# KKKSQJ/DeepLearning

Measured on AMD Instinct MI355X. Metric: images/sec, higher is better.
Workload: dtype bf16; 1 GPU; model=resnet50, global_batch=256, image_size=224, parallelism=dp1

## Files before the change

csrc/batchnorm.hip:

```cpp
#include "common.h"
#include "vec.h"

namespace dla {

__device__ __forceinline__ float bn_pre(float x, float sc, float sh) {
  return fmaf(x, sc, sh);
}

template <typename dev_t>
__global__ void bn_stats_kernel(const dev_t* __restrict__ x, float* __restrict__ sums,
                                int N, int C, int64_t HW) {
  __shared__ float smem[16];
  const int c = blockIdx.x;
  const int64_t total = (int64_t)N * HW;
  float sum = 0.f, sumsq = 0.f;
  for (int64_t m = (int64_t)blockIdx.y * blockDim.x + threadIdx.x; m < total;
       m += (int64_t)gridDim.y * blockDim.x) {
    const int64_t n = m / HW, hw = m % HW;
    const float f = to_f32(x[(n * C + c) * HW + hw]);
    sum += f;
    sumsq += f * f;
  }
  sum = block_reduce_sum(sum, smem);
  sumsq = block_reduce_sum(sumsq, smem);
// ... 153 lines not shown
    const float m_dyxh = sums[C + c] * inv_count;
    dx[i] = from_f32<dev_t>(weight[c] * rs * (g - m_dy - xh * m_dyxh));
  }
}



inline int64_t nhwc_used_threads(int lanes_per_row, int64_t rows,
                                 int64_t target_lanes) {
  int64_t k = target_lanes / lanes_per_row;
  if (k > rows) k = rows;
  if (k < 1) k = 1;
  return (int64_t)lanes_per_row * k;
}

template <typename dev_t, int V>
__global__ void bn_stats_nhwc_kernel(const dev_t* __restrict__ x,
                                     float* __restrict__ sums, int C,
                                     int64_t rows, int64_t used) {
  extern __shared__ float ls[];
  for (int i = threadIdx.x; i < 2 * C; i += blockDim.x) ls[i] = 0.f;
  __syncthreads();
  const int64_t t = (int64_t)blockIdx.x * blockDim.x + threadIdx.x;
  const int lanes_per_row = C / V;
  if (t < used) {
    const int c0 = (int)(t % lanes_per_row) * V;
    const int64_t rstride = used / lanes_per_row;
    float s[V], q[V];
#pragma unroll
    for (int j = 0; j < V; ++j) { s[j] = 0.f; q[j] = 0.f; }
    for (int64_t r = t / lanes_per_row; r < rows; r += rstride) {
      Vec<dev_t, V> xv = vload<dev_t, V>(x + r * C + c0);
#pragma unroll
      for (int j = 0; j < V; ++j) {
        const float f = to_f32(xv.v[j]);
        s[j] += f;
        q[j] += f * f;
      }
    }
#pragma unroll
    for (int j = 0; j < V; ++j) {
      atomicAdd(&ls[c0 + j], s[j]);
      atomicAdd(&ls[C + c0 + j], q[j]);
    }
  }
  __syncthreads();
  for (int i = threadIdx.x; i < 2 * C; i += blockDim.x)
    atomicAdd(&sums[i], ls[i]);
}

template <typename dev_t, int V, bool RELU>
__global__ void bn_apply_nhwc_kernel(const dev_t* __restrict__ x,
                                     const float* __restrict__ scale,
                                     const float* __restrict__ shift,
                                     dev_t* __restrict__ y, int C, int64_t rows,
                                     int64_t used) {
  const int64_t t = (int64_t)blockIdx.x * blockDim.x + threadIdx.x;
  if (t >= used) return;
  const int lanes_per_row = C / V;
  const int c0 = (int)(t % lanes_per_row) * V;
  const int64_t rstride = used / lanes_per_row;
  float sc[V], sh[V];
#pragma unroll
  for (int j = 0; j < V; ++j) { sc[j] = scale[c0 + j]; sh[j] = shift[c0 + j]; }
  for (int64_t r = t / lanes_per_row; r < rows; r += rstride) {
    Vec<dev_t, V> xv = vload<dev_t, V>(x + r * C + c0);
    Vec<dev_t, V> yv;
#pragma unroll
    for (int j = 0; j < V; ++j) {
      const float f = bn_pre(to_f32(xv.v[j]), sc[j], sh[j]);
      yv.v[j] = from_f32<dev_t>(RELU ? fmaxf(f, 0.f) : f);
    }
    vstore<dev_t, V>(y + r * C + c0, yv);
  }
}

template <typename dev_t, int V, bool RELU, bool MASK_Y = false>
__global__ void bn_bwd_stats_nhwc_kernel(const dev_t* __restrict__ dy,
                                         const dev_t* __restrict__ x,
                                         const dev_t* __restrict__ y,
                                         const float* __restrict__ scale,
                                         const float* __restrict__ shift,
                                         const float* __restrict__ mean,
                                         const float* __restrict__ rstd,
                                         float* __restrict__ sums, int C,
                                         int64_t rows, int64_t used) {
  extern __shared__ float ls[];
  for (int i = threadIdx.x; i < 2 * C; i += blockDim.x) ls[i] = 0.f;
  __syncthreads();
  const int64_t t = (int64_t)blockIdx.x * blockDim.x + threadIdx.x;
  const int lanes_per_row = C / V;
  if (t < used) {
    const int c0 = (int)(t % lanes_per_row) * V;
    const int64_t rstride = used / lanes_per_row;
    float mu[V], rs[V], sc[V], sh[V], s_dy[V], s_dyxh[V];
#pragma unroll
    for (int j = 0; j < V; ++j) {
      mu[j] = mean[c0 + j];
      rs[j] = rstd[c0 + j];
      sc[j] = (RELU && !MASK_Y) ? scale[c0 + j] : 0.f;
      sh[j] = (RELU && !MASK_Y) ? shift[c0 + j] : 0.f;
      s_dy[j] = 0.f;
      s_dyxh[j] = 0.f;
    }
    for (int64_t r = t / lanes_per_row; r < rows; r += rstride) {
      const int64_t base = r * C + c0;
      Vec<dev_t, V> dyv = vload<dev_t, V>(dy + base);
      Vec<dev_t, V> xv = vload<dev_t, V>(x + base);
      Vec<dev_t, V> yv;
      if (RELU && MASK_Y) yv = vload<dev_t, V>(y + base);
#pragma unroll
      for (int j = 0; j < V; ++j) {
        float g = to_f32(dyv.v[j]);
        const float xf = to_f32(xv.v[j]);
        if (RELU && MASK_Y && to_f32(yv.v[j]) <= 0.f) g = 0.f;
        if (RELU && !MASK_Y && !(bn_pre(xf, sc[j], sh[j]) > 0.f)) g = 0.f;
        const float xh = (xf - mu[j]) * rs[j];
        s_dy[j] += g;
        s_dyxh[j] += g * xh;
      }
    }
#pragma unroll
    for (int j = 0; j < V; ++j) {
      atomicAdd(&ls[c0 + j], s_dy[j]);
      atomicAdd(&ls[C + c0 + j], s_dyxh[j]);
    }
  }
  __syncthreads();
  for (int i = threadIdx.x; i < 2 * C; i += blockDim.x)
    atomicAdd(&sums[i], ls[i]);
}

template <typename dev_t, int V, bool RELU, bool MASK_Y = false>
__global__ void bn_bwd_dx_nhwc_kernel(const dev_t* __restrict__ dy,
                                      const dev_t* __restrict__ x,
                                      const dev_t* __restrict__ y,
                                      const float* __restrict__ scale,
                                      const float* __restrict__ shift,
                                      const float* __restrict__ mean,
                                      const float* __restrict__ rstd,
                                      const float* __restrict__ weight,
                                      const float* __restrict__ sums,
                                      dev_t* __restrict__ dx, int C,
                                      int64_t rows, int64_t used,
                                      float inv_count) {
// ... 61 lines not shown
    const int64_t base = r * C + c0;
    Vec<dev_t, V> xv = vload<dev_t, V>(x + base);
    Vec<dev_t, V> iv = vload<dev_t, V>(idn + base);
    Vec<dev_t, V> ov;
#pragma unroll
    for (int j = 0; j < V; ++j) {
      float f = to_f32(xv.v[j]) * sc[j] + sh[j];
      f += DUAL ? to_f32(iv.v[j]) * scd[j] : to_f32(iv.v[j]);
      ov.v[j] = from_f32<dev_t>(fmaxf(f, 0.f));
    }
    vstore<dev_t, V>(out + base, ov);
  }
}

template <typename dev_t, int V, bool DUAL>
__global__ void bn_join_bwd_stats_nhwc_kernel(
    const dev_t* __restrict__ dy, const dev_t* __restrict__ out,
    const dev_t* __restrict__ x, const float* __restrict__ mean,
    const float* __restrict__ rstd, const dev_t* __restrict__ xd,
    const float* __restrict__ mean_d, const float* __restrict__ rstd_d,
    dev_t* __restrict__ g_out, float* __restrict__ sums, int C, int64_t rows,
    int64_t used) {
  constexpr int NS = DUAL ? 3 : 2;
  extern __shared__ float ls[];
  for (int i = threadIdx.x; i < NS * C; i += blockDim.x) ls[i] = 0.f;
  __syncthreads();
  const int64_t t = (int64_t)blockIdx.x * blockDim.x + threadIdx.x;
  const int lanes_per_row = C / V;
  if (t < used) {
    const int c0 = (int)(t % lanes_per_row) * V;
    const int64_t rstride = used / lanes_per_row;
    float mu[V], rs[V], mud[V], rsd[V], s_g[V], s_gxh[V], s_gxhd[V];
#pragma unroll
    for (int j = 0; j < V; ++j) {
      mu[j] = mean[c0 + j];
      rs[j] = rstd[c0 + j];
      mud[j] = DUAL ? mean_d[c0 + j] : 0.f;
      rsd[j] = DUAL ? rstd_d[c0 + j] : 0.f;
      s_g[j] = 0.f;
      s_gxh[j] = 0.f;
      s_gxhd[j] = 0.f;
    }
    for (int64_t r = t / lanes_per_row; r < rows; r += rstride) {
      const int64_t base = r * C + c0;
      Vec<dev_t, V> dyv = vload<dev_t, V>(dy + base);
      Vec<dev_t, V> ov = vload<dev_t, V>(out + base);
      Vec<dev_t, V> xv = vload<dev_t, V>(x + base);
      Vec<dev_t, V> xdv;
      if (DUAL) xdv = vload<dev_t, V>(xd + base);
      Vec<dev_t, V> gv;
#pragma unroll
      for (int j = 0; j < V; ++j) {
        const bool on = to_f32(ov.v[j]) > 0.f;
        gv.v[j] = on ? dyv.v[j] : from_f32<dev_t>(0.f);
        const float g = on ? to_f32(dyv.v[j]) : 0.f;
        s_g[j] += g;
        s_gxh[j] += g * ((to_f32(xv.v[j]) - mu[j]) * rs[j]);
        if (DUAL) s_gxhd[j] += g * ((to_f32(xdv.v[j]) - mud[j]) * rsd[j]);
      }
      vstore<dev_t, V>(g_out + base, gv);
    }
#pragma unroll
    for (int j = 0; j < V; ++j) {
      atomicAdd(&ls[c0 + j], s_g[j]);
      atomicAdd(&ls[C + c0 + j], s_gxh[j]);
      if (DUAL) atomicAdd(&ls[2 * C + c0 + j], s_gxhd[j]);
    }
  }
  __syncthreads();
  for (int i = threadIdx.x; i < NS * C; i += blockDim.x)
    atomicAdd(&sums[i], ls[i]);
}

template <typename dev_t, int V>
__global__ void bn_join_bwd_dx_dual_nhwc_kernel(
    const dev_t* __restrict__ g, const dev_t* __restrict__ x,
    const dev_t* __restrict__ xd, const float* __restrict__ mean,
    const float* __restrict__ rstd, const float* __restrict__ weight,
    const float* __restrict__ mean_d, const float* __restrict__ rstd_d,
    const float* __restrict__ weight_d, const float* __restrict__ sums,
    dev_t* __restrict__ dx, dev_t* __restrict__ dxd, int C, int64_t rows,
    int64_t used, float inv_count) {
  const int64_t t = (int64_t)blockIdx.x * blockDim.x + threadIdx.x;
  if (t >= used) return;
  const int lanes_per_row = C / V;
  const int c0 = (int)(t % lanes_per_row) * V;
// ... 74 lines not shown
    hipLaunchKernelGGL(bn_finalize_kernel, dim3((C + 255) / 256), dim3(256), 0,
                       stream(), sums.data_ptr<float>(), w32.data_ptr<float>(),
                       b32.data_ptr<float>(), f.mean.data_ptr<float>(),
                       f.rstd.data_ptr<float>(), rm, rv,
                       f.scale.data_ptr<float>(), f.shift.data_ptr<float>(), C,
                       (float)rows, (float)eps, (float)momentum);
  }
  return f;
}

inline torch::Tensor bn_param_grad(const torch::Tensor& sums, int64_t offset,
                                   int C, const torch::Tensor& weight) {
  return sums.narrow(0, offset, C).to(weight.scalar_type());
}

inline bool is_nhwc_rows(const torch::Tensor& t) {
  return t.dim() == 4 && t.is_contiguous(at::MemoryFormat::ChannelsLast);
}

}

std::vector<torch::Tensor> batchnorm_fwd(torch::Tensor x, torch::Tensor weight,
                                         torch::Tensor bias,
                                         c10::optional<torch::Tensor> running_mean,
                                         c10::optional<torch::Tensor> running_var,
                                         double momentum, double eps, bool relu) {
  DLA_CHECK_CUDA(x);
  TORCH_CHECK(x.dim() == 4, "batchnorm_fwd expects a 4D tensor");
  const bool nhwc = dla::is_nhwc(x);
  TORCH_CHECK(nhwc || x.is_contiguous(), "batchnorm_fwd: x must be contiguous "
              "(NCHW or channels_last)");
  const int N = (int)x.size(0), C = (int)x.size(1);
  const int64_t HW = x.size(2) * x.size(3);
  auto opts_f = x.options().dtype(torch::kFloat);
  auto sums = torch::zeros({2 * C}, opts_f);
  auto mean = torch::empty({C}, opts_f);
  auto rstd = torch::empty({C}, opts_f);
  auto scale = torch::empty({C}, opts_f);
  auto shift = torch::empty({C}, opts_f);
  auto y = torch::empty_like(x);
  auto w32 = weight.to(torch::kFloat);
  auto b32 = bias.to(torch::kFloat);

  const int64_t rows = (int64_t)N * HW;
  const int ysplit = (int)std::min<int64_t>((rows + 65535) / 65536 + 1,
                                            std::max(1, 2048 / C));
  DLA_DISPATCH_FLOAT_TYPES(x.scalar_type(), "batchnorm_fwd", [&] {
    if (nhwc) {
      constexpr int VM = 16 / (int)sizeof(dev_t);
      auto stats = [&](auto vtag) {
        constexpr int V = decltype(vtag)::value;
        const int lanes = C / V;
        const int64_t used = dla::nhwc_used_threads(lanes, rows, 262144);
        const int lds = 2 * C * sizeof(float);
        hipLaunchKernelGGL((dla::bn_stats_nhwc_kernel<dev_t, V>),
                           dim3((int)((used + 255) / 256)), dim3(256), lds,
                           dla::stream(), (const dev_t*)x.data_ptr(),
                           sums.data_ptr<float>(), C, rows, used);
      };
      if (C % VM == 0) stats(std::integral_constant<int, VM>{});
      else if (C % 2 == 0) stats(std::integral_constant<int, 2>{});
      else stats(std::integral_constant<int, 1>{});
    } else {
      hipLaunchKernelGGL((dla::bn_stats_kernel<dev_t>), dim3(C, ysplit), dim3(256), 0,
                         dla::stream(), (const dev_t*)x.data_ptr(),
                         sums.data_ptr<float>(), N, C, HW);
    }
    hipLaunchKernelGGL(dla::bn_finalize_kernel, dim3((C + 255) / 256), dim3(256), 0,
                       dla::stream(), sums.data_ptr<float>(), w32.data_ptr<float>(),
                       b32.data_ptr<float>(), mean.data_ptr<float>(),
                       rstd.data_ptr<float>(),
                       running_mean.has_value() ? running_mean->data_ptr<float>() : nullptr,
                       running_var.has_value() ? running_var->data_ptr<float>() : nullptr,
                       scale.data_ptr<float>(), shift.data_ptr<float>(), C,
                       (float)rows, (float)eps, (float)momentum);
    const int64_t n_total = x.numel();
    constexpr int VMAX = 16 / (int)sizeof(dev_t);
    auto launch = [&](auto vtag, auto rtag) {
      constexpr int V = decltype(vtag)::value;
      constexpr bool R = decltype(rtag)::value;
      if (nhwc) {
        const int lanes = C / V;
        const int64_t used = dla::nhwc_used_threads(lanes, rows, 524288);
        hipLaunchKernelGGL((dla::bn_apply_nhwc_kernel<dev_t, V, R>),
                           dim3((int)((used + 255) / 256)), dim3(256), 0,
                           dla::stream(), (const dev_t*)x.data_ptr(),
                           scale.data_ptr<float>(), shift.data_ptr<float>(),
                           (dev_t*)y.data_ptr(), C, rows, used);
        return;
      }
// ... 127 lines not shown

std::vector<torch::Tensor> batchnorm_bwd_ex(
    torch::Tensor dy, torch::Tensor x, c10::optional<torch::Tensor> y,
    torch::Tensor weight, torch::Tensor mean, torch::Tensor rstd,
    c10::optional<torch::Tensor> scale, c10::optional<torch::Tensor> shift,
    bool relu) {
  DLA_CHECK_CUDA(dy); DLA_CHECK_CUDA(x);
  const bool nhwc = dla::is_nhwc(x);
  TORCH_CHECK(nhwc || x.is_contiguous(), "batchnorm_bwd: x must be contiguous");
  if (nhwc && !dla::is_nhwc(dy)) dy = dy.contiguous(at::MemoryFormat::ChannelsLast);
  if (!nhwc) dy = dy.contiguous();
  const int N = (int)x.size(0), C = (int)x.size(1);
  const int64_t HW = x.size(2) * x.size(3);
  const int64_t rows = (int64_t)N * HW;
  auto opts_f = x.options().dtype(torch::kFloat);
  auto sums = torch::zeros({2 * C}, opts_f);
  auto dx = torch::empty_like(x);
  auto w32 = weight.to(torch::kFloat);
  const int ysplit = (int)std::min<int64_t>((rows + 65535) / 65536 + 1,
                                            std::max(1, 2048 / C));
  const bool mask_y = relu && y.has_value();
  if (relu && !mask_y) {
    TORCH_CHECK(bn_relu_mask_from_x(x) && scale.has_value() && shift.has_value(),
                "batchnorm_bwd: the relu mask needs y, or channels_last x "
                "with the forward's scale and shift");
    for (const auto* t : {&*scale, &*shift})
      TORCH_CHECK(t->is_cuda() && t->scalar_type() == torch::kFloat &&
                      t->is_contiguous() && t->numel() == C,
                  "batchnorm_bwd: scale/shift must be contiguous fp32 [C]");
  }
  if (mask_y)
// ... 4 lines not shown
  const float* shp = (relu && !mask_y) ? shift->data_ptr<float>() : nullptr;
  DLA_DISPATCH_FLOAT_TYPES(x.scalar_type(), "batchnorm_bwd", [&] {
    const dev_t* yp = mask_y ? (const dev_t*)y->data_ptr() : nullptr;
    auto with_mode = [&](auto f) {
      if (!relu) f(std::false_type{}, std::false_type{});
      else if (mask_y) f(std::true_type{}, std::true_type{});
      else f(std::true_type{}, std::false_type{});
    };
    with_mode([&](auto rtag, auto mtag) {
      constexpr bool R = decltype(rtag)::value;
      constexpr bool MY = decltype(mtag)::value;
      if (nhwc) {
        constexpr int VM = 16 / (int)sizeof(dev_t);
        auto stats = [&](auto vtag) {
          constexpr int V = decltype(vtag)::value;
          const int lanes = C / V;
          const int64_t used = dla::nhwc_used_threads(lanes, rows, 262144);
          const int lds = 2 * C * sizeof(float);
          hipLaunchKernelGGL((dla::bn_bwd_stats_nhwc_kernel<dev_t, V, R, MY>),
                             dim3((int)((used + 255) / 256)), dim3(256), lds,
                             dla::stream(), (const dev_t*)dy.data_ptr(),
                             (const dev_t*)x.data_ptr(), yp, scp, shp,
                             mean.data_ptr<float>(), rstd.data_ptr<float>(),
                             sums.data_ptr<float>(), C, rows, used);
        };
        if (C % VM == 0) stats(std::integral_constant<int, VM>{});
        else if (C % 2 == 0) stats(std::integral_constant<int, 2>{});
        else stats(std::integral_constant<int, 1>{});
      } else if constexpr (!R || MY) {
        hipLaunchKernelGGL((dla::bn_bwd_stats_kernel<dev_t, R>), dim3(C, ysplit),
                           dim3(256), 0, dla::stream(), (const dev_t*)dy.data_ptr(),
                           (const dev_t*)x.data_ptr(), yp, mean.data_ptr<float>(),
                           rstd.data_ptr<float>(), sums.data_ptr<float>(), N, C, HW);
      }
    });

    const int64_t n_total = x.numel();
    const float inv_count = 1.f / (float)rows;
    constexpr int VMAX = 16 / (int)sizeof(dev_t);
// ... 121 lines not shown

std::vector<torch::Tensor> bn_add_relu_bwd(torch::Tensor dy, torch::Tensor out,
                                           torch::Tensor x, torch::Tensor weight,
                                           torch::Tensor mean,
                                           torch::Tensor rstd) {
  DLA_CHECK_CUDA(x);
  TORCH_CHECK(dla::is_nhwc_rows(x), "bn_add_relu_bwd: x must be channels_last");
  dla::join_check(x, out, "out");
  if (!dla::is_nhwc_rows(dy)) dy = dy.contiguous(at::MemoryFormat::ChannelsLast);
  dla::join_check(x, dy, "dy");
  dla::join_vec(x);
  const int C = (int)x.size(1);
  const int64_t rows = x.numel() / C;
  TORCH_CHECK(mean.numel() == C && rstd.numel() == C && weight.numel() == C,
              "bn_add_relu_bwd: per-channel tensors must have C elements");
  auto sums = torch::zeros({2 * C}, x.options().dtype(torch::kFloat));
  auto g = torch::empty_like(x);
  auto dx = torch::empty_like(x);
  auto w32 = weight.to(torch::kFloat).contiguous();
  DLA_DISPATCH_FLOAT_TYPES(x.scalar_type(), "bn_add_relu_bwd", [&] {
    constexpr int V = 16 / (int)sizeof(dev_t);
    const int lanes = C / V;
    const int64_t used_s = dla::nhwc_used_threads(lanes, rows, 262144);
    hipLaunchKernelGGL((dla::bn_join_bwd_stats_nhwc_kernel<dev_t, V, false>),
                       dim3((int)((used_s + 255) / 256)), dim3(256),
                       2 * C * sizeof(float), dla::stream(),
                       (const dev_t*)dy.data_ptr(), (const dev_t*)out.data_ptr(),
                       (const dev_t*)x.data_ptr(), mean.data_ptr<float>(),
                       rstd.data_ptr<float>(), nullptr, nullptr, nullptr,
                       (dev_t*)g.data_ptr(), sums.data_ptr<float>(), C, rows,
                       used_s);
    const int64_t used = dla::nhwc_used_threads(lanes, rows, 524288);
    hipLaunchKernelGGL((dla::bn_bwd_dx_nhwc_kernel<dev_t, V, false>),
                       dim3((int)((used + 255) / 256)), dim3(256), 0,
                       dla::stream(), (const dev_t*)g.data_ptr(),
                       (const dev_t*)x.data_ptr(), nullptr, nullptr, nullptr,
                       mean.data_ptr<float>(), rstd.data_ptr<float>(),
                       w32.data_ptr<float>(), sums.data_ptr<float>(),
                       (dev_t*)dx.data_ptr(), C, rows, used,
                       1.f / (float)rows);
  });
  HIP_CHECK_ERR();
  return {g, dx, dla::bn_param_grad(sums, C, C, weight),
          dla::bn_param_grad(sums, 0, C, weight)};
}

// ... 2 lines not shown
    torch::Tensor mean, torch::Tensor rstd, torch::Tensor xd,
    torch::Tensor weight_d, torch::Tensor mean_d, torch::Tensor rstd_d) {
  DLA_CHECK_CUDA(x);
  TORCH_CHECK(dla::is_nhwc_rows(x), "bn_add_relu_dual_bwd: x must be channels_last");
  dla::join_check(x, out, "out");
  dla::join_check(x, xd, "xd");
  if (!dla::is_nhwc_rows(dy)) dy = dy.contiguous(at::MemoryFormat::ChannelsLast);
  dla::join_check(x, dy, "dy");
  dla::join_vec(x);
  const int C = (int)x.size(1);
  const int64_t rows = x.numel() / C;
  TORCH_CHECK(mean.numel() == C && rstd.numel() == C && weight.numel() == C &&
                  mean_d.numel() == C && rstd_d.numel() == C &&
                  weight_d.numel() == C,
              "bn_add_relu_dual_bwd: per-channel tensors must have C elements");
  auto sums = torch::zeros({3 * C}, x.options().dtype(torch::kFloat));
  auto g = torch::empty_like(x);
  auto dx = torch::empty_like(x);
  auto dxd = torch::empty_like(x);
  auto w32 = weight.to(torch::kFloat).contiguous();
  auto wd32 = weight_d.to(torch::kFloat).contiguous();
  DLA_DISPATCH_FLOAT_TYPES(x.scalar_type(), "bn_add_relu_dual_bwd", [&] {
    constexpr int V = 16 / (int)sizeof(dev_t);
    const int lanes = C / V;
    const int64_t used_s = dla::nhwc_used_threads(lanes, rows, 262144);
    hipLaunchKernelGGL((dla::bn_join_bwd_stats_nhwc_kernel<dev_t, V, true>),
                       dim3((int)((used_s + 255) / 256)), dim3(256),
                       3 * C * sizeof(float), dla::stream(),
                       (const dev_t*)dy.data_ptr(), (const dev_t*)out.data_ptr(),
                       (const dev_t*)x.data_ptr(), mean.data_ptr<float>(),
                       rstd.data_ptr<float>(), (const dev_t*)xd.data_ptr(),
                       mean_d.data_ptr<float>(), rstd_d.data_ptr<float>(),
                       (dev_t*)g.data_ptr(), sums.data_ptr<float>(), C, rows,
                       used_s);
    const int64_t used = dla::nhwc_used_threads(lanes, rows, 524288);
    hipLaunchKernelGGL((dla::bn_join_bwd_dx_dual_nhwc_kernel<dev_t, V>),
                       dim3((int)((used + 255) / 256)), dim3(256), 0,
                       dla::stream(), (const dev_t*)g.data_ptr(),
                       (const dev_t*)x.data_ptr(), (const dev_t*)xd.data_ptr(),
                       mean.data_ptr<float>(), rstd.data_ptr<float>(),
                       w32.data_ptr<float>(), mean_d.data_ptr<float>(),
                       rstd_d.data_ptr<float>(), wd32.data_ptr<float>(),
                       sums.data_ptr<float>(), (dev_t*)dx.data_ptr(),
                       (dev_t*)dxd.data_ptr(), C, rows, used,
                       1.f / (float)rows);
  });
  HIP_CHECK_ERR();
  auto dbias = dla::bn_param_grad(sums, 0, C, weight);
  return {dx, dxd, dla::bn_param_grad(sums, C, C, weight), dbias,
// ... 81 lines not shown
    for (int ow = w >> 1; ow <= ow_hi; ++ow) {
      const int want = kh * 3 + (w - 2 * ow + 1);
      const int64_t o = (((int64_t)n * OH + oh) * OW + ow) * C + c0;
      Vec<uint8_t, V> sv = vload<uint8_t, V>(slots + o);
      Vec<dev_t, V> dv = vload<dev_t, V>(dpool + o);
#pragma unroll
      for (int j = 0; j < V; ++j)
        if ((int)sv.v[j] == want) g[j] += to_f32(dv.v[j]);
    }
  }
#pragma unroll
  for (int j = 0; j < V; ++j)
    if (!(bn_pre(to_f32(xv.v[j]), sc[j], sh[j]) > 0.f)) g[j] = 0.f;
}

template <typename dev_t, int V>
__global__ void bn_relu_maxpool_bwd_stats_nhwc_kernel(
    const dev_t* __restrict__ dpool, const uint8_t* __restrict__ slots,
    const dev_t* __restrict__ x, const float* __restrict__ scale,
    const float* __restrict__ shift, const float* __restrict__ mean,
    const float* __restrict__ rstd, float* __restrict__ sums, int C, int H,
    int W, int OH, int OW, int64_t rows, int64_t used) {
  extern __shared__ float ls[];
  for (int i = threadIdx.x; i < 2 * C; i += blockDim.x) ls[i] = 0.f;
  __syncthreads();
  const int64_t t = (int64_t)blockIdx.x * blockDim.x + threadIdx.x;
  const int lanes_per_row = C / V;
  if (t < used) {
    const int c0 = (int)(t % lanes_per_row) * V;
    const int64_t rstride = used / lanes_per_row;
    float mu[V], rs[V], sc[V], sh[V], s_g[V], s_gxh[V], g[V];
#pragma unroll
    for (int j = 0; j < V; ++j) {
      mu[j] = mean[c0 + j];
      rs[j] = rstd[c0 + j];
      sc[j] = scale[c0 + j];
      sh[j] = shift[c0 + j];
      s_g[j] = 0.f;
      s_gxh[j] = 0.f;
    }
    for (int64_t r = t / lanes_per_row; r < rows; r += rstride) {
      const uint32_t r32 = (uint32_t)r;
      const uint32_t q = r32 / (uint32_t)W;
      const int w = (int)(r32 - q * (uint32_t)W);
      const int n = (int)(q / (uint32_t)H);
      const int h = (int)(q - (uint32_t)n * (uint32_t)H);
      Vec<dev_t, V> xv = vload<dev_t, V>(x + r * C + c0);
      stem_pool_grad<dev_t, V>(dpool, slots, xv, sc, sh, n, h, w, c0, C, OH,
                               OW, g);
#pragma unroll
      for (int j = 0; j < V; ++j) {
        const float xh = (to_f32(xv.v[j]) - mu[j]) * rs[j];
        s_g[j] += g[j];
        s_gxh[j] += g[j] * xh;
      }
    }
#pragma unroll
    for (int j = 0; j < V; ++j) {
      atomicAdd(&ls[c0 + j], s_g[j]);
      atomicAdd(&ls[C + c0 + j], s_gxh[j]);
    }
  }
  __syncthreads();
  for (int i = threadIdx.x; i < 2 * C; i += blockDim.x)
    atomicAdd(&sums[i], ls[i]);
}

template <typename dev_t, int V>
__global__ void bn_relu_maxpool_bwd_dx_nhwc_kernel(
    const dev_t* __restrict__ dpool, const uint8_t* __restrict__ slots,
    const dev_t* __restrict__ x, const float* __restrict__ scale,
    const float* __restrict__ shift, const float* __restrict__ mean,
    const float* __restrict__ rstd, const float* __restrict__ weight,
    const float* __restrict__ sums, dev_t* __restrict__ dx, int C, int H,
    int W, int OH, int OW, int64_t rows, int64_t used, float inv_count) {
  const int64_t t = (int64_t)blockIdx.x * blockDim.x + threadIdx.x;
  if (t >= used) return;
  const int lanes_per_row = C / V;
  const int c0 = (int)(t % lanes_per_row) * V;
  const int64_t rstride = used / lanes_per_row;
// ... 35 lines not shown
  TORCH_CHECK(x.numel() > 0 && x.numel() / x.size(1) < (int64_t(1) << 31),
              fn, ": N*H*W must be in [1, 2^31)");
}

}

std::vector<torch::Tensor> bn_relu_maxpool_fwd(
    torch::Tensor x, torch::Tensor weight, torch::Tensor bias,
    c10::optional<torch::Tensor> running_mean,
    c10::optional<torch::Tensor> running_var, double momentum, double eps) {
  dla::stem_check(x, "bn_relu_maxpool_fwd");
  const int N = (int)x.size(0), C = (int)x.size(1);
  const int H = (int)x.size(2), W = (int)x.size(3);
  const int OH = (H - 1) / 2 + 1, OW = (W - 1) / 2 + 1;
  const int64_t rows = (int64_t)N * H * W;
  auto sums = torch::zeros({2 * C}, x.options().dtype(torch::kFloat));
  auto out_opts = x.options().memory_format(at::MemoryFormat::ChannelsLast);
  auto pooled = torch::empty({N, C, OH, OW}, out_opts);
  auto slots = torch::empty({N, C, OH, OW}, out_opts.dtype(torch::kByte));
  const int runs = (OH + dla::kPoolRun - 1) / dla::kPoolRun;
  TORCH_CHECK((int64_t)N * runs < (int64_t(1) << 31),
              "bn_relu_maxpool_fwd: too many blocks");
  dla::BnFinalized fin;
  DLA_DISPATCH_FLOAT_TYPES(x.scalar_type(), "bn_relu_maxpool_fwd", [&] {
    constexpr int V = 16 / (int)sizeof(dev_t);
    const int64_t used = dla::nhwc_used_threads(C / V, rows, 262144);
    hipLaunchKernelGGL((dla::bn_stats_nhwc_kernel<dev_t, V>),
                       dim3((int)((used + 255) / 256)), dim3(256),
                       2 * C * sizeof(float), dla::stream(),
                       (const dev_t*)x.data_ptr(), sums.data_ptr<float>(), C,
                       rows, used);
    fin = dla::bn_finalize_launch(sums, weight, bias, running_mean,
                                  running_var, C, rows, momentum, eps);
    hipLaunchKernelGGL((dla::bn_relu_maxpool_fwd_nhwc_kernel<dev_t, V>),
                       dim3(N * runs), dim3(256), 0, dla::stream(),
                       (const dev_t*)x.data_ptr(), fin.scale.data_ptr<float>(),
                       fin.shift.data_ptr<float>(), (dev_t*)pooled.data_ptr(),
                       slots.data_ptr<uint8_t>(), C, H, W, OH, OW, runs);
  });
  HIP_CHECK_ERR();
  return {pooled, slots, fin.mean, fin.rstd, fin.scale, fin.shift};
}

std::vector<torch::Tensor> bn_relu_maxpool_bwd(
    torch::Tensor dpool, torch::Tensor x, torch::Tensor slots,
    torch::Tensor weight, torch::Tensor mean, torch::Tensor rstd,
// ... 9 lines not shown
  const std::vector<int64_t> pshape{N, C, OH, OW};
  TORCH_CHECK(dpool.scalar_type() == x.scalar_type() &&
                  dpool.sizes() == at::IntArrayRef(pshape),
              "bn_relu_maxpool_bwd: dpool must be [N, C, OH, OW] of x's dtype");
  TORCH_CHECK(slots.is_cuda() && slots.scalar_type() == torch::kByte &&
                  slots.sizes() == at::IntArrayRef(pshape) &&
                  dla::is_nhwc_rows(slots),
              "bn_relu_maxpool_bwd: slots must be channels_last uint8 "
              "[N, C, OH, OW]");
  for (const auto* t : {&mean, &rstd, &scale, &shift})
    TORCH_CHECK(t->is_cuda() && t->scalar_type() == torch::kFloat &&
                    t->is_contiguous() && t->numel() == C,
                "bn_relu_maxpool_bwd: per-channel tensors must be contiguous "
                "fp32 [C]");
  TORCH_CHECK(weight.numel() == C, "bn_relu_maxpool_bwd: weight must be [C]");
  auto sums = torch::zeros({2 * C}, x.options().dtype(torch::kFloat));
  auto dx = torch::empty_like(x);
  auto w32 = weight.to(torch::kFloat).contiguous();
  DLA_DISPATCH_FLOAT_TYPES(x.scalar_type(), "bn_relu_maxpool_bwd", [&] {
    constexpr int V = 16 / (int)sizeof(dev_t);
    const int lanes = C / V;
    const int64_t used_s = dla::nhwc_used_threads(lanes, rows, 262144);
    hipLaunchKernelGGL((dla::bn_relu_maxpool_bwd_stats_nhwc_kernel<dev_t, V>),
                       dim3((int)((used_s + 255) / 256)), dim3(256),
                       2 * C * sizeof(float), dla::stream(),
                       (const dev_t*)dpool.data_ptr(),
                       slots.data_ptr<uint8_t>(), (const dev_t*)x.data_ptr(),
                       scale.data_ptr<float>(), shift.data_ptr<float>(),
                       mean.data_ptr<float>(), rstd.data_ptr<float>(),
                       sums.data_ptr<float>(), C, H, W, OH, OW, rows, used_s);
    const int64_t used = dla::nhwc_used_threads(lanes, rows, 524288);
    hipLaunchKernelGGL((dla::bn_relu_maxpool_bwd_dx_nhwc_kernel<dev_t, V>),
                       dim3((int)((used + 255) / 256)), dim3(256), 0,
                       dla::stream(), (const dev_t*)dpool.data_ptr(),
                       slots.data_ptr<uint8_t>(), (const dev_t*)x.data_ptr(),
                       scale.data_ptr<float>(), shift.data_ptr<float>(),
                       mean.data_ptr<float>(), rstd.data_ptr<float>(),
                       w32.data_ptr<float>(), sums.data_ptr<float>(),
                       (dev_t*)dx.data_ptr(), C, H, W, OH, OW, rows, used,
                       1.f / (float)rows);
  });
  HIP_CHECK_ERR();
  return {dx, dla::bn_param_grad(sums, C, C, weight),
          dla::bn_param_grad(sums, 0, C, weight)};
}
// ... 1 lines not shown
```

Before: 9196 images/s.

## Replace atomic BN channel reductions with two-stage slab reduction

```diff
diff --git a/csrc/batchnorm.hip b/csrc/batchnorm.hip
--- a/csrc/batchnorm.hip
+++ b/csrc/batchnorm.hip
@@ -191,39 +191,138 @@
   return (int64_t)lanes_per_row * k;
 }
 
+constexpr int kRedThreads = 256;
+constexpr int kRedLanes = 32;
+constexpr int kRedBlocks = 2048;
+constexpr int kRedMaxParts = 512;
+constexpr int kRedMinRows = 8;
+constexpr int red_unroll(int tensors) { return tensors <= 2 ? 4 : 2; }
+
+#define DLA_RED_KERNEL \
+  __launch_bounds__(dla::kRedThreads) __attribute__((amdgpu_waves_per_eu(1, 4)))
+
+struct NhwcRedTile {
+  int bl, rb, chunks, parts;
+};
+
+inline NhwcRedTile nhwc_red_tile(int lanes_per_row, int64_t rows,
+                                 int blocks = kRedBlocks,
+                                 int max_parts = kRedMaxParts) {
+  NhwcRedTile t;
+  t.chunks = (lanes_per_row + kRedLanes - 1) / kRedLanes;
+  t.bl = (lanes_per_row + t.chunks - 1) / t.chunks;
+  t.rb = kRedThreads / t.bl;
+  const int64_t per_part = (int64_t)t.rb * kRedMinRows;
+  const int64_t by_rows = (rows + per_part - 1) / per_part;
+  const int64_t p = std::min<int64_t>(
+      std::min<int64_t>(blocks / t.chunks, max_parts), by_rows);
+  t.parts = (int)std::max<int64_t>(p, 1);
+  return t;
+}
+
+struct NhwcRedPos {
+  int c0;
+  int64_t row;
+  int64_t rstride;
+  bool active;
+};
+
+template <int V>
+__device__ __forceinline__ NhwcRedPos nhwc_red_pos(int C, int bl, int rb) {
+  const int lane = threadIdx.x % bl, rl = threadIdx.x / bl;
+  const int gl = blockIdx.x * bl + lane;
+  NhwcRedPos p;
+  p.c0 = gl * V;
+  p.row = (int64_t)blockIdx.y * rb + rl;
+  p.rstride = (int64_t)gridDim.y * rb;
+  p.active = rl < rb && gl < C / V;
+  return p;
+}
+
+template <int U, typename L, typename A>
+__device__ __forceinline__ void nhwc_red_rows(const NhwcRedPos& p,
+                                              int64_t rows, L&& load, A&& add) {
+  if (!p.active) return;
+  using D = decltype(load(int64_t{}));
+  int64_t r = p.row;
+  for (; r + (U - 1) * p.rstride < rows; r += U * p.rstride) {
+    D d[U];
+#pragma unroll
+    for (int u = 0; u < U; ++u) d[u] = load(r + u * p.rstride);
+#pragma unroll
+    for (int u = 0; u < U; ++u) add(r + u * p.rstride, d[u]);
+  }
+  for (; r < rows; r += p.rstride) add(r, load(r));
+}
+
+template <int V, int NS>
+__device__ __forceinline__ void nhwc_red_tail(const float (&acc)[NS][V],
+                                              float* __restrict__ slab, int C,
+                                              int bl, int rb) {
+  __shared__ __attribute__((aligned(16))) float ls[kRedThreads * V];
+  const int W = bl * V;
+  const int cbase = blockIdx.x * W;
+  float* out = slab + (int64_t)blockIdx.y * NS * C;
+#pragma unroll
+  for (int s = 0; s < NS; ++s) {
+    if (s) __syncthreads();
+    if ((int)threadIdx.x < bl * rb) {
+#pragma unroll
+      for (int j = 0; j < V; ++j) ls[threadIdx.x * V + j] = acc[s][j];
+    }
+    __syncthreads();
+    for (int col = threadIdx.x; col < W; col += kRedThreads) {
+      if (cbase + col < C) {
+        float sum = 0.f;
+        for (int r = 0; r < rb; ++r) sum += ls[r * W + col];
+        out[s * C + cbase + col] = sum;
+      }
+    }
+  }
+}
+
+constexpr int kSlabCols = 32, kSlabRows = 32;
+
+__global__ void __launch_bounds__(kSlabCols * kSlabRows)
+bn_slab_reduce_kernel(const float* __restrict__ slab, int n_parts, int n_cols,
+                      float* __restrict__ sums) {
+  __shared__ float ls[kSlabRows][kSlabCols + 1];
+  const int cl = threadIdx.x % kSlabCols, rl = threadIdx.x / kSlabCols;
+  const int c = blockIdx.x * kSlabCols + cl;
+  float s = 0.f;
+  if (c < n_cols) {
+#pragma unroll 4
+    for (int r = rl; r < n_parts; r += kSlabRows)
+      s += slab[(int64_t)r * n_cols + c];
+  }
+  ls[rl][cl] = s;
+  __syncthreads();
+  for (int h = kSlabRows / 2; h > 0; h >>= 1) {
+    if (rl < h) ls[rl][cl] += ls[rl + h][cl];
+    __syncthreads();
+  }
+  if (rl == 0 && c < n_cols) sums[c] = ls[0][cl];
+}
+
 template <typename dev_t, int V>
-__global__ void bn_stats_nhwc_kernel(const dev_t* __restrict__ x,
-                                     float* __restrict__ sums, int C,
-                                     int64_t rows, int64_t used) {
-  extern __shared__ float ls[];
-  for (int i = threadIdx.x; i < 2 * C; i += blockDim.x) ls[i] = 0.f;
-  __syncthreads();
-  const int64_t t = (int64_t)blockIdx.x * blockDim.x + threadIdx.x;
-  const int lanes_per_row = C / V;
-  if (t < used) {
-    const int c0 = (int)(t % lanes_per_row) * V;
-    const int64_t rstride = used / lanes_per_row;
-    float s[V], q[V];
-#pragma unroll
-    for (int j = 0; j < V; ++j) { s[j] = 0.f; q[j] = 0.f; }
-    for (int64_t r = t / lanes_per_row; r < rows; r += rstride) {
-      Vec<dev_t, V> xv = vload<dev_t, V>(x + r * C + c0);
-#pragma unroll
-      for (int j = 0; j < V; ++j) {
-        const float f = to_f32(xv.v[j]);
-        s[j] += f;
-        q[j] += f * f;
-      }
-    }
-#pragma unroll
-    for (int j = 0; j < V; ++j) {
-      atomicAdd(&ls[c0 + j], s[j]);
-      atomicAdd(&ls[C + c0 + j], q[j]);
-    }
-  }
-  __syncthreads();
-  for (int i = threadIdx.x; i < 2 * C; i += blockDim.x)
-    atomicAdd(&sums[i], ls[i]);
+__global__ void DLA_RED_KERNEL
+bn_stats_nhwc_kernel(const dev_t* __restrict__ x, float* __restrict__ slab,
+                     int C, int64_t rows, int bl, int rb) {
+  const NhwcRedPos p = nhwc_red_pos<V>(C, bl, rb);
+  float acc[2][V];
+#pragma unroll
+  for (int j = 0; j < V; ++j) { acc[0][j] = 0.f; acc[1][j] = 0.f; }
+  nhwc_red_rows<red_unroll(1)>(
+      p, rows, [&](int64_t r) { return vload<dev_t, V>(x + r * C + p.c0); },
+      [&](int64_t, const Vec<dev_t, V>& xv) {
+#pragma unroll
+        for (int j = 0; j < V; ++j) {
+          const float f = to_f32(xv.v[j]);
+          acc[0][j] += f;
+          acc[1][j] += f * f;
+        }
+      });
+  nhwc_red_tail<V, 2>(acc, slab, C, bl, rb);
 }
 
 template <typename dev_t, int V, bool RELU>
@@ -253,59 +352,54 @@
 }
 
 template <typename dev_t, int V, bool RELU, bool MASK_Y = false>
-__global__ void bn_bwd_stats_nhwc_kernel(const dev_t* __restrict__ dy,
-                                         const dev_t* __restrict__ x,
-                                         const dev_t* __restrict__ y,
-                                         const float* __restrict__ scale,
-                                         const float* __restrict__ shift,
-                                         const float* __restrict__ mean,
-                                         const float* __restrict__ rstd,
-                                         float* __restrict__ sums, int C,
-                                         int64_t rows, int64_t used) {
-  extern __shared__ float ls[];
-  for (int i = threadIdx.x; i < 2 * C; i += blockDim.x) ls[i] = 0.f;
-  __syncthreads();
-  const int64_t t = (int64_t)blockIdx.x * blockDim.x + threadIdx.x;
-  const int lanes_per_row = C / V;
-  if (t < used) {
-    const int c0 = (int)(t % lanes_per_row) * V;
-    const int64_t rstride = used / lanes_per_row;
-    float mu[V], rs[V], sc[V], sh[V], s_dy[V], s_dyxh[V];
-#pragma unroll
-    for (int j = 0; j < V; ++j) {
-      mu[j] = mean[c0 + j];
-      rs[j] = rstd[c0 + j];
-      sc[j] = (RELU && !MASK_Y) ? scale[c0 + j] : 0.f;
-      sh[j] = (RELU && !MASK_Y) ? shift[c0 + j] : 0.f;
-      s_dy[j] = 0.f;
-      s_dyxh[j] = 0.f;
-    }
-    for (int64_t r = t / lanes_per_row; r < rows; r += rstride) {
-      const int64_t base = r * C + c0;
-      Vec<dev_t, V> dyv = vload<dev_t, V>(dy + base);
-      Vec<dev_t, V> xv = vload<dev_t, V>(x + base);
-      Vec<dev_t, V> yv;
-      if (RELU && MASK_Y) yv = vload<dev_t, V>(y + base);
-#pragma unroll
-      for (int j = 0; j < V; ++j) {
-        float g = to_f32(dyv.v[j]);
-        const float xf = to_f32(xv.v[j]);
-        if (RELU && MASK_Y && to_f32(yv.v[j]) <= 0.f) g = 0.f;
-        if (RELU && !MASK_Y && !(bn_pre(xf, sc[j], sh[j]) > 0.f)) g = 0.f;
-        const float xh = (xf - mu[j]) * rs[j];
-        s_dy[j] += g;
-        s_dyxh[j] += g * xh;
-      }
-    }
-#pragma unroll
-    for (int j = 0; j < V; ++j) {
-      atomicAdd(&ls[c0 + j], s_dy[j]);
-      atomicAdd(&ls[C + c0 + j], s_dyxh[j]);
-    }
-  }
-  __syncthreads();
-  for (int i = threadIdx.x; i < 2 * C; i += blockDim.x)
-    atomicAdd(&sums[i], ls[i]);
+__global__ void DLA_RED_KERNEL
+bn_bwd_stats_nhwc_kernel(const dev_t* __restrict__ dy,
+                         const dev_t* __restrict__ x,
+                         const dev_t* __restrict__ y,
+                         const float* __restrict__ scale,
+                         const float* __restrict__ shift,
+                         const float* __restrict__ mean,
+                         const float* __restrict__ rstd,
+                         float* __restrict__ slab, int C, int64_t rows, int bl,
+                         int rb) {
+  const NhwcRedPos p = nhwc_red_pos<V>(C, bl, rb);
+  float mu[V], rs[V], sc[V], sh[V];
+  float acc[2][V];
+#pragma unroll
+  for (int j = 0; j < V; ++j) {
+    mu[j] = p.active ? mean[p.c0 + j] : 0.f;
+    rs[j] = p.active ? rstd[p.c0 + j] : 0.f;
+    sc[j] = (p.active && RELU && !MASK_Y) ? scale[p.c0 + j] : 0.f;
+    sh[j] = (p.active && RELU && !MASK_Y) ? shift[p.c0 + j] : 0.f;
+    acc[0][j] = 0.f;
+    acc[1][j] = 0.f;
+  }
+  struct Row {
+    Vec<dev_t, V> dy, x, y;
+  };
+  nhwc_red_rows<red_unroll(MASK_Y ? 3 : 2)>(
+      p, rows,
+      [&](int64_t r) {
+        const int64_t base = r * C + p.c0;
+        Row d;
+        d.dy = vload<dev_t, V>(dy + base);
+        d.x = vload<dev_t, V>(x + base);
+        if (RELU && MASK_Y) d.y = vload<dev_t, V>(y + base);
+        return d;
+      },
+      [&](int64_t, const Row& d) {
+#pragma unroll
+        for (int j = 0; j < V; ++j) {
+          float g = to_f32(d.dy.v[j]);
+          const float xf = to_f32(d.x.v[j]);
+          if (RELU && MASK_Y && to_f32(d.y.v[j]) <= 0.f) g = 0.f;
+          if (RELU && !MASK_Y && !(bn_pre(xf, sc[j], sh[j]) > 0.f)) g = 0.f;
+          const float xh = (xf - mu[j]) * rs[j];
+          acc[0][j] += g;
+          acc[1][j] += g * xh;
+        }
+      });
+  nhwc_red_tail<V, 2>(acc, slab, C, bl, rb);
 }
 
 template <typename dev_t, int V, bool RELU, bool MASK_Y = false>
@@ -397,62 +491,56 @@
 }
 
 template <typename dev_t, int V, bool DUAL>
-__global__ void bn_join_bwd_stats_nhwc_kernel(
+__global__ void DLA_RED_KERNEL
+bn_join_bwd_stats_nhwc_kernel(
     const dev_t* __restrict__ dy, const dev_t* __restrict__ out,
     const dev_t* __restrict__ x, const float* __restrict__ mean,
     const float* __restrict__ rstd, const dev_t* __restrict__ xd,
     const float* __restrict__ mean_d, const float* __restrict__ rstd_d,
-    dev_t* __restrict__ g_out, float* __restrict__ sums, int C, int64_t rows,
-    int64_t used) {
+    dev_t* __restrict__ g_out, float* __restrict__ slab, int C, int64_t rows,
+    int bl, int rb) {
   constexpr int NS = DUAL ? 3 : 2;
-  extern __shared__ float ls[];
-  for (int i = threadIdx.x; i < NS * C; i += blockDim.x) ls[i] = 0.f;
-  __syncthreads();
-  const int64_t t = (int64_t)blockIdx.x * blockDim.x + threadIdx.x;
-  const int lanes_per_row = C / V;
-  if (t < used) {
-    const int c0 = (int)(t % lanes_per_row) * V;
-    const int64_t rstride = used / lanes_per_row;
-    float mu[V], rs[V], mud[V], rsd[V], s_g[V], s_gxh[V], s_gxhd[V];
-#pragma unroll
-    for (int j = 0; j < V; ++j) {
-      mu[j] = mean[c0 + j];
-      rs[j] = rstd[c0 + j];
-      mud[j] = DUAL ? mean_d[c0 + j] : 0.f;
-      rsd[j] = DUAL ? rstd_d[c0 + j] : 0.f;
-      s_g[j] = 0.f;
-      s_gxh[j] = 0.f;
-      s_gxhd[j] = 0.f;
-    }
-    for (int64_t r = t / lanes_per_row; r < rows; r += rstride) {
-      const int64_t base = r * C + c0;
-      Vec<dev_t, V> dyv = vload<dev_t, V>(dy + base);
-      Vec<dev_t, V> ov = vload<dev_t, V>(out + base);
-      Vec<dev_t, V> xv = vload<dev_t, V>(x + base);
-      Vec<dev_t, V> xdv;
-      if (DUAL) xdv = vload<dev_t, V>(xd + base);
-      Vec<dev_t, V> gv;
-#pragma unroll
-      for (int j = 0; j < V; ++j) {
-        const bool on = to_f32(ov.v[j]) > 0.f;
-        gv.v[j] = on ? dyv.v[j] : from_f32<dev_t>(0.f);
-        const float g = on ? to_f32(dyv.v[j]) : 0.f;
-        s_g[j] += g;
-        s_gxh[j] += g * ((to_f32(xv.v[j]) - mu[j]) * rs[j]);
-        if (DUAL) s_gxhd[j] += g * ((to_f32(xdv.v[j]) - mud[j]) * rsd[j]);
-      }
-      vstore<dev_t, V>(g_out + base, gv);
-    }
-#pragma unroll
-    for (int j = 0; j < V; ++j) {
-      atomicAdd(&ls[c0 + j], s_g[j]);
-      atomicAdd(&ls[C + c0 + j], s_gxh[j]);
-      if (DUAL) atomicAdd(&ls[2 * C + c0 + j], s_gxhd[j]);
-    }
-  }
-  __syncthreads();
-  for (int i = threadIdx.x; i < NS * C; i += blockDim.x)
-    atomicAdd(&sums[i], ls[i]);
+  const NhwcRedPos p = nhwc_red_pos<V>(C, bl, rb);
+  float mu[V], rs[V], mud[V], rsd[V];
+  float acc[NS][V];
+#pragma unroll
+  for (int j = 0; j < V; ++j) {
+    mu[j] = p.active ? mean[p.c0 + j] : 0.f;
+    rs[j] = p.active ? rstd[p.c0 + j] : 0.f;
+    mud[j] = (p.active && DUAL) ? mean_d[p.c0 + j] : 0.f;
+    rsd[j] = (p.active && DUAL) ? rstd_d[p.c0 + j] : 0.f;
+#pragma unroll
+    for (int s = 0; s < NS; ++s) acc[s][j] = 0.f;
+  }
+  struct Row {
+    Vec<dev_t, V> dy, out, x, xd;
+  };
+  nhwc_red_rows<red_unroll(DUAL ? 4 : 3)>(
+      p, rows,
+      [&](int64_t r) {
+        const int64_t base = r * C + p.c0;
+        Row d;
+        d.dy = vload<dev_t, V>(dy + base);
+        d.out = vload<dev_t, V>(out + base);
+        d.x = vload<dev_t, V>(x + base);
+        if (DUAL) d.xd = vload<dev_t, V>(xd + base);
+        return d;
+      },
+      [&](int64_t r, const Row& d) {
+        Vec<dev_t, V> gv;
+#pragma unroll
+        for (int j = 0; j < V; ++j) {
+          const bool on = to_f32(d.out.v[j]) > 0.f;
+          gv.v[j] = on ? d.dy.v[j] : from_f32<dev_t>(0.f);
+          const float g = on ? to_f32(d.dy.v[j]) : 0.f;
+          acc[0][j] += g;
+          acc[1][j] += g * ((to_f32(d.x.v[j]) - mu[j]) * rs[j]);
+          if (DUAL)
+            acc[NS - 1][j] += g * ((to_f32(d.xd.v[j]) - mud[j]) * rsd[j]);
+        }
+        vstore<dev_t, V>(g_out + r * C + p.c0, gv);
+      });
+  nhwc_red_tail<V, NS>(acc, slab, C, bl, rb);
 }
 
 template <typename dev_t, int V>
@@ -557,6 +645,17 @@
   return sums.narrow(0, offset, C).to(weight.scalar_type());
 }
 
+inline torch::Tensor bn_slab_reduce_launch(const torch::Tensor& slab) {
+  const int n_parts = (int)slab.size(0), n_cols = (int)slab.size(1);
+  auto sums = torch::empty({n_cols}, slab.options());
+  hipLaunchKernelGGL(bn_slab_reduce_kernel,
+                     dim3((n_cols + kSlabCols - 1) / kSlabCols),
+                     dim3(kSlabCols * kSlabRows), 0, stream(),
+                     slab.data_ptr<float>(), n_parts, n_cols,
+                     sums.data_ptr<float>());
+  return sums;
+}
+
 inline bool is_nhwc_rows(const torch::Tensor& t) {
   return t.dim() == 4 && t.is_contiguous(at::MemoryFormat::ChannelsLast);
 }
@@ -576,7 +675,7 @@
   const int N = (int)x.size(0), C = (int)x.size(1);
   const int64_t HW = x.size(2) * x.size(3);
   auto opts_f = x.options().dtype(torch::kFloat);
-  auto sums = torch::zeros({2 * C}, opts_f);
+  auto sums = nhwc ? torch::Tensor() : torch::zeros({2 * C}, opts_f);
   auto mean = torch::empty({C}, opts_f);
   auto rstd = torch::empty({C}, opts_f);
   auto scale = torch::empty({C}, opts_f);
@@ -593,13 +692,12 @@
       constexpr int VM = 16 / (int)sizeof(dev_t);
       auto stats = [&](auto vtag) {
         constexpr int V = decltype(vtag)::value;
-        const int lanes = C / V;
-        const int64_t used = dla::nhwc_used_threads(lanes, rows, 262144);
-        const int lds = 2 * C * sizeof(float);
+        const auto t = dla::nhwc_red_tile(C / V, rows);
+        sums = torch::empty({t.parts, 2 * C}, opts_f);
         hipLaunchKernelGGL((dla::bn_stats_nhwc_kernel<dev_t, V>),
-                           dim3((int)((used + 255) / 256)), dim3(256), lds,
+                           dim3(t.chunks, t.parts), dim3(dla::kRedThreads), 0,
                            dla::stream(), (const dev_t*)x.data_ptr(),
-                           sums.data_ptr<float>(), C, rows, used);
+                           sums.data_ptr<float>(), C, rows, t.bl, t.rb);
       };
       if (C % VM == 0) stats(std::integral_constant<int, VM>{});
       else if (C % 2 == 0) stats(std::integral_constant<int, 2>{});
@@ -609,14 +707,25 @@
                          dla::stream(), (const dev_t*)x.data_ptr(),
                          sums.data_ptr<float>(), N, C, HW);
     }
-    hipLaunchKernelGGL(dla::bn_finalize_kernel, dim3((C + 255) / 256), dim3(256), 0,
-                       dla::stream(), sums.data_ptr<float>(), w32.data_ptr<float>(),
-                       b32.data_ptr<float>(), mean.data_ptr<float>(),
-                       rstd.data_ptr<float>(),
-                       running_mean.has_value() ? running_mean->data_ptr<float>() : nullptr,
-                       running_var.has_value() ? running_var->data_ptr<float>() : nullptr,
-                       scale.data_ptr<float>(), shift.data_ptr<float>(), C,
-                       (float)rows, (float)eps, (float)momentum);
+    float* rm = running_mean.has_value() ? running_mean->data_ptr<float>() : nullptr;
+    float* rv = running_var.has_value() ? running_var->data_ptr<float>() : nullptr;
+    if (sums.dim() == 2 && sums.size(0) > 1) {
+      hipLaunchKernelGGL(dla::bn_finalize_parts_kernel,
+                         dim3((C + dla::kFinCh - 1) / dla::kFinCh),
+                         dim3(dla::kFinCh * dla::kFinRows), 0, dla::stream(),
+                         sums.data_ptr<float>(), (int)sums.size(0),
+                         w32.data_ptr<float>(), b32.data_ptr<float>(),
+                         mean.data_ptr<float>(), rstd.data_ptr<float>(), rm, rv,
+                         scale.data_ptr<float>(), shift.data_ptr<float>(), C,
+                         (float)rows, (float)eps, (float)momentum);
+    } else {
+      hipLaunchKernelGGL(dla::bn_finalize_kernel, dim3((C + 255) / 256), dim3(256), 0,
+                         dla::stream(), sums.data_ptr<float>(), w32.data_ptr<float>(),
+                         b32.data_ptr<float>(), mean.data_ptr<float>(),
+                         rstd.data_ptr<float>(), rm, rv,
+                         scale.data_ptr<float>(), shift.data_ptr<float>(), C,
+                         (float)rows, (float)eps, (float)momentum);
+    }
     const int64_t n_total = x.numel();
     constexpr int VMAX = 16 / (int)sizeof(dev_t);
     auto launch = [&](auto vtag, auto rtag) {
@@ -774,7 +883,7 @@
   const int64_t HW = x.size(2) * x.size(3);
   const int64_t rows = (int64_t)N * HW;
   auto opts_f = x.options().dtype(torch::kFloat);
-  auto sums = torch::zeros({2 * C}, opts_f);
+  auto sums = nhwc ? torch::Tensor() : torch::zeros({2 * C}, opts_f);
   auto dx = torch::empty_like(x);
   auto w32 = weight.to(torch::kFloat);
   const int ysplit = (int)std::min<int64_t>((rows + 65535) / 65536 + 1,
@@ -809,15 +918,15 @@
         constexpr int VM = 16 / (int)sizeof(dev_t);
         auto stats = [&](auto vtag) {
           constexpr int V = decltype(vtag)::value;
-          const int lanes = C / V;
-          const int64_t used = dla::nhwc_used_threads(lanes, rows, 262144);
-          const int lds = 2 * C * sizeof(float);
+          const auto t = dla::nhwc_red_tile(C / V, rows);
+          auto slab = torch::empty({t.parts, 2 * C}, opts_f);
           hipLaunchKernelGGL((dla::bn_bwd_stats_nhwc_kernel<dev_t, V, R, MY>),
-                             dim3((int)((used + 255) / 256)), dim3(256), lds,
-                             dla::stream(), (const dev_t*)dy.data_ptr(),
+                             dim3(t.chunks, t.parts), dim3(dla::kRedThreads),
+                             0, dla::stream(), (const dev_t*)dy.data_ptr(),
                              (const dev_t*)x.data_ptr(), yp, scp, shp,
                              mean.data_ptr<float>(), rstd.data_ptr<float>(),
-                             sums.data_ptr<float>(), C, rows, used);
+                             slab.data_ptr<float>(), C, rows, t.bl, t.rb);
+          sums = dla::bn_slab_reduce_launch(slab);
         };
         if (C % VM == 0) stats(std::integral_constant<int, VM>{});
         else if (C % 2 == 0) stats(std::integral_constant<int, 2>{});
@@ -969,22 +1078,25 @@
   const int64_t rows = x.numel() / C;
   TORCH_CHECK(mean.numel() == C && rstd.numel() == C && weight.numel() == C,
               "bn_add_relu_bwd: per-channel tensors must have C elements");
-  auto sums = torch::zeros({2 * C}, x.options().dtype(torch::kFloat));
+  torch::Tensor sums;
   auto g = torch::empty_like(x);
   auto dx = torch::empty_like(x);
   auto w32 = weight.to(torch::kFloat).contiguous();
   DLA_DISPATCH_FLOAT_TYPES(x.scalar_type(), "bn_add_relu_bwd", [&] {
     constexpr int V = 16 / (int)sizeof(dev_t);
     const int lanes = C / V;
-    const int64_t used_s = dla::nhwc_used_threads(lanes, rows, 262144);
+    const auto t = dla::nhwc_red_tile(lanes, rows);
+    auto slab = torch::empty({t.parts, 2 * C},
+                             x.options().dtype(torch::kFloat));
     hipLaunchKernelGGL((dla::bn_join_bwd_stats_nhwc_kernel<dev_t, V, false>),
-                       dim3((int)((used_s + 255) / 256)), dim3(256),
-                       2 * C * sizeof(float), dla::stream(),
+                       dim3(t.chunks, t.parts), dim3(dla::kRedThreads), 0,
+                       dla::stream(),
                        (const dev_t*)dy.data_ptr(), (const dev_t*)out.data_ptr(),
                        (const dev_t*)x.data_ptr(), mean.data_ptr<float>(),
                        rstd.data_ptr<float>(), nullptr, nullptr, nullptr,
-                       (dev_t*)g.data_ptr(), sums.data_ptr<float>(), C, rows,
-                       used_s);
+                       (dev_t*)g.data_ptr(), slab.data_ptr<float>(), C, rows,
+                       t.bl, t.rb);
+    sums = dla::bn_slab_reduce_launch(slab);
     const int64_t used = dla::nhwc_used_threads(lanes, rows, 524288);
     hipLaunchKernelGGL((dla::bn_bwd_dx_nhwc_kernel<dev_t, V, false>),
                        dim3((int)((used + 255) / 256)), dim3(256), 0,
@@ -1017,7 +1129,7 @@
                   mean_d.numel() == C && rstd_d.numel() == C &&
                   weight_d.numel() == C,
               "bn_add_relu_dual_bwd: per-channel tensors must have C elements");
-  auto sums = torch::zeros({3 * C}, x.options().dtype(torch::kFloat));
+  torch::Tensor sums;
   auto g = torch::empty_like(x);
   auto dx = torch::empty_like(x);
   auto dxd = torch::empty_like(x);
@@ -1026,16 +1138,19 @@
   DLA_DISPATCH_FLOAT_TYPES(x.scalar_type(), "bn_add_relu_dual_bwd", [&] {
     constexpr int V = 16 / (int)sizeof(dev_t);
     const int lanes = C / V;
-    const int64_t used_s = dla::nhwc_used_threads(lanes, rows, 262144);
+    const auto t = dla::nhwc_red_tile(lanes, rows);
+    auto slab = torch::empty({t.parts, 3 * C},
+                             x.options().dtype(torch::kFloat));
     hipLaunchKernelGGL((dla::bn_join_bwd_stats_nhwc_kernel<dev_t, V, true>),
-                       dim3((int)((used_s + 255) / 256)), dim3(256),
-                       3 * C * sizeof(float), dla::stream(),
+                       dim3(t.chunks, t.parts), dim3(dla::kRedThreads), 0,
+                       dla::stream(),
                        (const dev_t*)dy.data_ptr(), (const dev_t*)out.data_ptr(),
                        (const dev_t*)x.data_ptr(), mean.data_ptr<float>(),
                        rstd.data_ptr<float>(), (const dev_t*)xd.data_ptr(),
                        mean_d.data_ptr<float>(), rstd_d.data_ptr<float>(),
-                       (dev_t*)g.data_ptr(), sums.data_ptr<float>(), C, rows,
-                       used_s);
+                       (dev_t*)g.data_ptr(), slab.data_ptr<float>(), C, rows,
+                       t.bl, t.rb);
+    sums = dla::bn_slab_reduce_launch(slab);
     const int64_t used = dla::nhwc_used_threads(lanes, rows, 524288);
     hipLaunchKernelGGL((dla::bn_join_bwd_dx_dual_nhwc_kernel<dev_t, V>),
                        dim3((int)((used + 255) / 256)), dim3(256), 0,
@@ -1147,56 +1262,47 @@
     if (!(bn_pre(to_f32(xv.v[j]), sc[j], sh[j]) > 0.f)) g[j] = 0.f;
 }
 
+constexpr int kStemRedBlocks = 1024;
+
 template <typename dev_t, int V>
-__global__ void bn_relu_maxpool_bwd_stats_nhwc_kernel(
+__global__ void __launch_bounds__(kRedThreads)
+bn_relu_maxpool_bwd_stats_nhwc_kernel(
     const dev_t* __restrict__ dpool, const uint8_t* __restrict__ slots,
     const dev_t* __restrict__ x, const float* __restrict__ scale,
     const float* __restrict__ shift, const float* __restrict__ mean,
-    const float* __restrict__ rstd, float* __restrict__ sums, int C, int H,
-    int W, int OH, int OW, int64_t rows, int64_t used) {
-  extern __shared__ float ls[];
-  for (int i = threadIdx.x; i < 2 * C; i += blockDim.x) ls[i] = 0.f;
-  __syncthreads();
-  const int64_t t = (int64_t)blockIdx.x * blockDim.x + threadIdx.x;
-  const int lanes_per_row = C / V;
-  if (t < used) {
-    const int c0 = (int)(t % lanes_per_row) * V;
-    const int64_t rstride = used / lanes_per_row;
-    float mu[V], rs[V], sc[V], sh[V], s_g[V], s_gxh[V], g[V];
-#pragma unroll
-    for (int j = 0; j < V; ++j) {
-      mu[j] = mean[c0 + j];
-      rs[j] = rstd[c0 + j];
-      sc[j] = scale[c0 + j];
-      sh[j] = shift[c0 + j];
-      s_g[j] = 0.f;
-      s_gxh[j] = 0.f;
-    }
-    for (int64_t r = t / lanes_per_row; r < rows; r += rstride) {
-      const uint32_t r32 = (uint32_t)r;
-      const uint32_t q = r32 / (uint32_t)W;
-      const int w = (int)(r32 - q * (uint32_t)W);
-      const int n = (int)(q / (uint32_t)H);
-      const int h = (int)(q - (uint32_t)n * (uint32_t)H);
-      Vec<dev_t, V> xv = vload<dev_t, V>(x + r * C + c0);
-      stem_pool_grad<dev_t, V>(dpool, slots, xv, sc, sh, n, h, w, c0, C, OH,
-                               OW, g);
-#pragma unroll
-      for (int j = 0; j < V; ++j) {
-        const float xh = (to_f32(xv.v[j]) - mu[j]) * rs[j];
-        s_g[j] += g[j];
-        s_gxh[j] += g[j] * xh;
-      }
-    }
-#pragma unroll
-    for (int j = 0; j < V; ++j) {
-      atomicAdd(&ls[c0 + j], s_g[j]);
-      atomicAdd(&ls[C + c0 + j], s_gxh[j]);
-    }
-  }
-  __syncthreads();
-  for (int i = threadIdx.x; i < 2 * C; i += blockDim.x)
-    atomicAdd(&sums[i], ls[i]);
+    const float* __restrict__ rstd, float* __restrict__ slab, int C, int H,
+    int W, int OH, int OW, int64_t rows, int bl, int rb) {
+  const NhwcRedPos p = nhwc_red_pos<V>(C, bl, rb);
+  float mu[V], rs[V], sc[V], sh[V];
+  float acc[2][V];
+#pragma unroll
+  for (int j = 0; j < V; ++j) {
+    mu[j] = p.active ? mean[p.c0 + j] : 0.f;
+    rs[j] = p.active ? rstd[p.c0 + j] : 0.f;
+    sc[j] = p.active ? scale[p.c0 + j] : 0.f;
+    sh[j] = p.active ? shift[p.c0 + j] : 0.f;
+    acc[0][j] = 0.f;
+    acc[1][j] = 0.f;
+  }
+  nhwc_red_rows<1>(
+      p, rows, [&](int64_t r) { return vload<dev_t, V>(x + r * C + p.c0); },
+      [&](int64_t r, const Vec<dev_t, V>& xv) {
+        const uint32_t r32 = (uint32_t)r;
+        const uint32_t q = r32 / (uint32_t)W;
+        const int w = (int)(r32 - q * (uint32_t)W);
+        const int n = (int)(q / (uint32_t)H);
+        const int h = (int)(q - (uint32_t)n * (uint32_t)H);
+        float g[V];
+        stem_pool_grad<dev_t, V>(dpool, slots, xv, sc, sh, n, h, w, p.c0, C,
+                                 OH, OW, g);
+#pragma unroll
+        for (int j = 0; j < V; ++j) {
+          const float xh = (to_f32(xv.v[j]) - mu[j]) * rs[j];
+          acc[0][j] += g[j];
+          acc[1][j] += g[j] * xh;
+        }
+      });
+  nhwc_red_tail<V, 2>(acc, slab, C, bl, rb);
 }
 
 template <typename dev_t, int V>
@@ -1262,7 +1368,6 @@
   const int H = (int)x.size(2), W = (int)x.size(3);
   const int OH = (H - 1) / 2 + 1, OW = (W - 1) / 2 + 1;
   const int64_t rows = (int64_t)N * H * W;
-  auto sums = torch::zeros({2 * C}, x.options().dtype(torch::kFloat));
   auto out_opts = x.options().memory_format(at::MemoryFormat::ChannelsLast);
   auto pooled = torch::empty({N, C, OH, OW}, out_opts);
   auto slots = torch::empty({N, C, OH, OW}, out_opts.dtype(torch::kByte));
@@ -1272,12 +1377,13 @@
   dla::BnFinalized fin;
   DLA_DISPATCH_FLOAT_TYPES(x.scalar_type(), "bn_relu_maxpool_fwd", [&] {
     constexpr int V = 16 / (int)sizeof(dev_t);
-    const int64_t used = dla::nhwc_used_threads(C / V, rows, 262144);
+    const auto t = dla::nhwc_red_tile(C / V, rows);
+    auto sums = torch::empty({t.parts, 2 * C},
+                             x.options().dtype(torch::kFloat));
     hipLaunchKernelGGL((dla::bn_stats_nhwc_kernel<dev_t, V>),
-                       dim3((int)((used + 255) / 256)), dim3(256),
-                       2 * C * sizeof(float), dla::stream(),
-                       (const dev_t*)x.data_ptr(), sums.data_ptr<float>(), C,
-                       rows, used);
+                       dim3(t.chunks, t.parts), dim3(dla::kRedThreads), 0,
+                       dla::stream(), (const dev_t*)x.data_ptr(),
+                       sums.data_ptr<float>(), C, rows, t.bl, t.rb);
     fin = dla::bn_finalize_launch(sums, weight, bias, running_mean,
                                   running_var, C, rows, momentum, eps);
     hipLaunchKernelGGL((dla::bn_relu_maxpool_fwd_nhwc_kernel<dev_t, V>),
@@ -1317,21 +1423,25 @@
                 "bn_relu_maxpool_bwd: per-channel tensors must be contiguous "
                 "fp32 [C]");
   TORCH_CHECK(weight.numel() == C, "bn_relu_maxpool_bwd: weight must be [C]");
-  auto sums = torch::zeros({2 * C}, x.options().dtype(torch::kFloat));
+  torch::Tensor sums;
   auto dx = torch::empty_like(x);
   auto w32 = weight.to(torch::kFloat).contiguous();
   DLA_DISPATCH_FLOAT_TYPES(x.scalar_type(), "bn_relu_maxpool_bwd", [&] {
     constexpr int V = 16 / (int)sizeof(dev_t);
     const int lanes = C / V;
-    const int64_t used_s = dla::nhwc_used_threads(lanes, rows, 262144);
+    const auto t = dla::nhwc_red_tile(lanes, rows, dla::kStemRedBlocks,
+                                      dla::kStemRedBlocks);
+    auto slab = torch::empty({t.parts, 2 * C},
+                             x.options().dtype(torch::kFloat));
     hipLaunchKernelGGL((dla::bn_relu_maxpool_bwd_stats_nhwc_kernel<dev_t, V>),
-                       dim3((int)((used_s + 255) / 256)), dim3(256),
-                       2 * C * sizeof(float), dla::stream(),
-                       (const dev_t*)dpool.data_ptr(),
+                       dim3(t.chunks, t.parts), dim3(dla::kRedThreads), 0,
+                       dla::stream(), (const dev_t*)dpool.data_ptr(),
                        slots.data_ptr<uint8_t>(), (const dev_t*)x.data_ptr(),
                        scale.data_ptr<float>(), shift.data_ptr<float>(),
                        mean.data_ptr<float>(), rstd.data_ptr<float>(),
-                       sums.data_ptr<float>(), C, H, W, OH, OW, rows, used_s);
+                       slab.data_ptr<float>(), C, H, W, OH, OW, rows, t.bl,
+                       t.rb);
+    sums = dla::bn_slab_reduce_launch(slab);
     const int64_t used = dla::nhwc_used_threads(lanes, rows, 524288);
     hipLaunchKernelGGL((dla::bn_relu_maxpool_bwd_dx_nhwc_kernel<dev_t, V>),
                        dim3((int)((used + 255) / 256)), dim3(256), 0,
```

New measurement: 9810 images/s (median of 6 runs). +6.7%, better.
